# tsai0507/PolishPathPlanning

Measured on AMD Instinct MI355X. Metric: polishing waypoints/sec for 1M-pt cloud, 256 slices; path L2 err vs ref, higher is better.
Workload: dtype f32; 1 GPU; cfg2_1m_s256; points_per_workpiece=999912, slices=256, waypoints_per_workpiece=25908, workpieces=1, batch_per_gpu=1, parallelism=single GPU, pairing=kd, walk=center_int (connect), dynamic_adjustment=False, handles_taking_turns=3

## Files before the change

### polishpathplanning_amd/csrc/ppp_engine.hip

```cpp
#include "ppp_kernels.h"
#ifdef PPP_SINGLE_TU
#include "ppp_window.h"
#endif
#include "ppp_handle.h"
#include "ppp_gather.h"
#include <atomic>
#include <cerrno>
#include <fcntl.h>
#include <thread>
#include <unistd.h>
#ifndef PPP_NN_HINT_SPACINGS
#define PPP_NN_HINT_SPACINGS 3.0
#endif
#ifndef PPP_SLAB_PTS
#define PPP_SLAB_PTS 832
#endif
#ifndef PPP_PPT8_FROM
#define PPP_PPT8_FROM 500000
#endif
#ifndef WIN_SLICE_WAVES_PER_CU
#define WIN_SLICE_WAVES_PER_CU 16
#endif
#ifndef PPP_WIN_PPT8_FROM
#define PPP_WIN_PPT8_FROM 1200000
// ... 324 lines not shown
    if (!capw) return PPP_OK;
    h->win_NBc_thr = std::max(16, NBc / 2);
    while (h->win_NBc_thr * 2 <= NBc && h->win_NBc_thr < expect / 10.0) h->win_NBc_thr <<= 1;
    if (const char *ev = tuning_env("PPP_WIN_NBC_THR")) { const int v = atoi(ev); if (v >= 16 && v <= NBc && (v & (v - 1)) == 0) h->win_NBc_thr = v; }
    const int NB = WIN_CLASSES * NBc;
    h->win_el_expect = max_el;
    h->win_capw = capw; h->win_cap_el = cap_el; h->win_NB = NB; h->win_NBc = NBc;
    int T = win_pick_threads(h, std::max(1, h->se - h->sb));
    if (!T) return PPP_OK;
    h->win_ppt_alone = n_src > PPP_WIN_PPT8_FROM ? 8 : 4;
    {
        int from = PPP_PPT16_FROM;
        if (const char *ev = tuning_env("PPP_WIN_STAGE_FROM")) from = atoi(ev);
        h->win_staged = n_src > from && !tuning_env("PPP_WIN_NO_STAGE");
    }
    if (h->win_staged) {
        h->win_ppt_alone = 8;
        if (win_scatter_lds_bytes(S, 8, WSC_T, true) + 2048 > (size_t)h->max_lds) h->win_ppt_alone = 4;
        if (win_scatter_lds_bytes(S, h->win_ppt_alone, WSC_T, true) + 2048 > (size_t)h->max_lds) { h->win_staged = false; h->win_ppt_alone = 8; }
    }
    win_pick_scatter(h, std::max(1, h->se - h->sb), n_src);
    h->win_gs = std::max(1, (n_src + h->win_ppt * h->win_scat_threads - 1) / (h->win_ppt * h->win_scat_threads));
    if (h->win_staged) h->win_gs = std::min(h->win_gs, std::max(1, h->num_cus));
    h->win_pad = pad; h->win_capw = capw; h->win_cap_el = cap_el; h->win_NB = NB; h->win_NBc = NBc; h->win_threads = T;
    h->win_stride = std::max(1, (int)per);
    h->win_rec_lds = (h->win_stride <= cap_el / 7) ? cap_el / 7 : 0;
#ifdef WIN_REC_GLOBAL
    h->win_rec_lds = 0;
#endif
    h->win_first_kept = h->P.drop_ends ? 1 : 0;
    h->win_nkept = std::max(0, h->P.drop_ends ? S - 2 : S);
    h->win_px0 = px[0];
    HIPCHK(h, h->win_part.ensure((size_t)std::max(h->win_gs, (n_src + 2 * 256 - 1) / (2 * 256))));
    HIPCHK(h, h->win_pts.ensure((size_t)S * (size_t)capw));
    {
        const double need = (double)S * (double)cap_el;
        if (need > 1.0e9) return PPP_OK;
        h->node_cap = std::max(h->node_cap, (int)need);
        HIPCHK(h, h->node_x.ensure(h->node_cap)); HIPCHK(h, h->node_y.ensure(h->node_cap)); HIPCHK(h, h->node_z.ensure(h->node_cap));
    }
    const size_t slots = (size_t)std::max(1, h->win_nkept) * (size_t)h->win_stride;
    HIPCHK(h, h->wps_xyz.ensure(slots)); HIPCHK(h, h->wps_normal.ensure(slots)); HIPCHK(h, h->wps_nn.ensure(slots)); HIPCHK(h, h->wps_pre.ensure(6 * slots)); HIPCHK(h, h->wps_rec.ensure(4 * slots));
    if (!from_auto && !inherit)
        HIPCHK(h, hipMemsetAsync(h->win_cnt.p, 0, sizeof(int) * (size_t)S * std::max<size_t>(3, WIN_CNT_STRIDE), h->stream));
    h->win_path = true;
    if (!inherit && h->sb == 0 && h->se == S && !h->use_part) {
        h->inh_valid = true; h->inh_S = S; h->inh_n = n_src; h->inh_max_w = max_w; h->inh_max_el = max_el; h->inh_pad = pad; h->inh_P = h->P;
    }
    if (getenv("PPP_WIN_DEBUG"))
        fprintf(stderr, "[ppp] window plan: S %d [%d,%d) pad %.2f capw %d cap_el %d NBc %d (throughput %d) threads %d ppt %d x %d threads lds %zu B max window %d max left side %d census %s\n",
                S, h->sb, h->se, pad, capw, cap_el, NBc, h->win_NBc_thr, T, h->win_ppt, h->win_scat_threads, win_slice_lds_for(h, NBc), max_w, max_el,
                from_auto ? "came with the cloud" : (inherit ? "inherited from an earlier cloud of this size" : "at plan time"));
    return PPP_OK;
}

static WinArgs win_args(const ppp_handle h)
{
    WinArgs A;
    memset(&A, 0, sizeof(A));
    A.m = h->meta.p; A.P = dev_params(h);
    A.X = h->use_part ? h->Xp.p : h->X.p; A.Y = h->use_part ? h->Yp.p : h->Y.p; A.Z = h->use_part ? h->Zp.p : h->Z.p;
    A.idmap = h->use_part ? h->part_idx.p : ((h->part_given && h->part_has_idx) ? h->part_idx.p : nullptr);
    A.n = h->use_part ? h->n_part : (int)h->n;
    A.plan_px = h->win_px.p;
    A.S = h->S_cap; A.sb = h->sb; A.se = h->se; A.first_kept = h->win_first_kept; A.nkept = h->win_nkept;
    A.pad = h->win_pad; A.px0 = h->win_px0; A.inv_step = 1.0f / (float)std::max(1, (int)(h->P.tool_radius * 2));
    A.y0 = h->h_mn[1];
    { const float yr = h->h_mx[1] - h->h_mn[1]; A.yscale = yr > 0.f ? (float)h->win_NBc / yr : 0.f; }
    for (int d = 0; d < 3; ++d) { A.plan_mn[d] = h->h_mn[d]; A.plan_mx[d] = h->h_mx[d]; }
    A.plan_nvalid = h->h_nvalid;
    A.capw = h->win_capw; A.cap_el = h->win_cap_el; A.NB = h->win_NB; A.NBc = h->win_NBc; A.stride = h->win_stride; A.rec_lds = h->win_rec_lds;
    A.W_cap = h->W_cap; A.node_cap = h->node_cap;
    A.g_scatter = h->win_gs; A.g_slice = std::max(0, h->se - h->sb); A.g_finish = h->sm_tiles;
    A.finish = h->ranged ? 0 : 1;
    A.win_cnt = h->win_cnt.p; A.win_pts = h->win_pts.p; A.win_part = h->win_part.p;
    A.px = h->px.p; A.lo = h->lo.p; A.hi = h->hi.p;
    A.node_x = h->node_x.p; A.node_y = h->node_y.p; A.node_z = h->node_z.p;
    A.node_start = h->node_start.p; A.node_cnt = h->node_cnt.p; A.band_cnt = h->band_cnt.p;
    A.wp_cnt = h->wp_cnt.p; A.wp_off = h->wp_off.p; A.tail = h->tail.p;
    A.wps_xyz = h->wps_xyz.p; A.wps_normal = h->wps_normal.p; A.wps_nn = h->wps_nn.p; A.wps_pre = h->wps_pre.p; A.wps_rec = h->wps_rec.p;
    A.wp_pre = h->wp_pre.p; A.wp_smooth = h->wp_smooth.p; A.wp_out = h->wp_out.p; A.out2 = h->out2; A.out2_cap = h->out2_cap;
    A.plan_rec = (h->rec_current && h->plan_walk_ok) ? h->plan_auto.p : nullptr;
    A.meta_host = h->hmeta_pinned.p; A.fin_ticket = h->fin_ticket.p;
    return A;
}
static size_t win_slice_lds(const ppp_handle h) { return win_slice_lds_for(h, h->win_NBc); }
static void win_args_throughput(const ppp_handle h, WinArgs &A)
{
    A.NBc = h->win_NBc_thr; A.NB = WIN_CLASSES * A.NBc;
    const float yr = h->h_mx[1] - h->h_mn[1];
    A.yscale = yr > 0.f ? (float)A.NBc / yr : 0.f;
}

static int enqueue_window_gen(ppp_handle h)
{
    WinArgs A = win_args(h);
    const bool thr = win_throughput_launch(h, A.g_slice);
    if (thr) win_args_throughput(h, A);
    const size_t scat_lds = win_scatter_lds_bytes(A.S, h->win_ppt, h->win_scat_threads, h->win_staged);
    if (h->win_scat_threads != WSC_T) {
        const int rcn = with_narrow_scatter(h->win_scat_threads, h->win_ppt, [&](auto ppt, auto st) -> int {
            LAUNCH(h, "k_win_scatter", (k_win_scatter<decltype(ppt)::value, false, decltype(st)::value>), A.g_scatter, decltype(st)::value, scat_lds, A);
            return PPP_OK;
        });
        if (rcn) return rcn;
    }
    else if (h->win_staged && h->win_ppt == 8) LAUNCH(h, "k_win_scatter", (k_win_scatter<8, true>), A.g_scatter, WSC_T, scat_lds, A);
    else if (h->win_staged) LAUNCH(h, "k_win_scatter", (k_win_scatter<4, true>), A.g_scatter, WSC_T, scat_lds, A);
    else if (h->win_ppt == 8) LAUNCH(h, "k_win_scatter", (k_win_scatter<8, false>), A.g_scatter, WSC_T, scat_lds, A);
    else if (h->win_ppt == 2) LAUNCH(h, "k_win_scatter", (k_win_scatter<2, false>), A.g_scatter, WSC_T, scat_lds, A);
    else LAUNCH(h, "k_win_scatter", (k_win_scatter<4, false>), A.g_scatter, WSC_T, scat_lds, A);
    const int T = h->win_threads;
    const size_t lds = win_slice_lds_for(h, A.NBc);
    const int extra = tuning_env("PPP_WIN_NO_VERIFY") ? 0 : 1;
    return with_block_size(T, [&](auto bs) -> int {
        LAUNCH(h, "k_win_slice", k_win_slice<decltype(bs)::value>, A.g_slice + extra, T, lds, A);
        return PPP_OK;
    });
}
static int enqueue_window_finish(ppp_handle h)
{
    const WinArgs A = win_args(h);
    LAUNCH(h, "k_win_finish", k_win_finish, A.g_finish, SMF_T, sizeof(int) * ((size_t)A.nkept + 2), A);
    return PPP_OK;
}

static int make_plan(ppp_handle h)
{
    if (!h->have_cloud) return fail(h, PPP_ERR_ARG, "no cloud set");
    h->pass.withdraw_plan();
    h->drop_graph();
    const int n = (int)h->n;
    int S = h->h_nvalid ? ppp_slice_walk(h->P.walk, h->h_mn[0], h->h_mx[0], h->P.tool_radius, nullptr, 0) : 0;
    if (S >= PPP_WALK_HARD_MAX) return fail(h, PPP_ERR_CAPACITY, "slice walk does not terminate");
    h->sb = std::min(std::max(0, h->P.slice_begin), S);
    h->se = (h->P.slice_end <= 0 || h->P.slice_end > S) ? S : h->P.slice_end;
    h->ranged = S > 0 && (h->sb > 0 || h->se < S);
    h->incl_lo = -INFINITY; h->incl_hi = INFINITY;
    h->n_range = h->h_nvalid;
    if (h->ranged) {
        if (h->sb >= h->se) { h->incl_lo = INFINITY; h->incl_hi = -INFINITY; h->n_range = 0; }
        else {
            std::vector<float> px((size_t)S);
            ppp_slice_walk(h->P.walk, h->h_mn[0], h->h_mx[0], h->P.tool_radius, px.data(), S);
            h->incl_lo = (float)((int)px[h->sb] - 2) - h->P.range_margin;
            h->incl_hi = (float)((int)px[h->se - 1] + 2) + h->P.range_margin;
            const double range = (double)h->h_mx[0] - (double)h->h_mn[0];
            const double part = std::min((double)h->incl_hi, (double)h->h_mx[0]) - std::max((double)h->incl_lo, (double)h->h_mn[0]);
            h->n_range = range > 0 ? (int)std::min((double)h->h_nvalid, std::max(0.0, part / range) * h->h_nvalid * 1.05 + 64) : h->h_nvalid;
        }
    }
    h->use_part = false; h->n_part = 0;
    if (h->part_given) {
        if (!h->ranged && !(h->part_lo == -INFINITY && h->part_hi == INFINITY))
            return fail(h, PPP_ERR_ARG, "a part-only cloud (ppp_set_cloud_part) needs a slice range: set slice_begin / slice_end");
        if (h->sb < h->se && !(h->incl_lo >= h->part_lo && h->incl_hi <= h->part_hi))
            return fail(h, PPP_ERR_ARG, "the slice range with its margin reaches beyond the part this handle was given (ppp_range_interval tells what it needs)");
        h->n_range = n;
    } else if (h->ranged && h->sb < h->se && n > 0) {
        const int nblocks = (n + COMPACT_CHUNK - 1) / COMPACT_CHUNK;
        DevBuf<int> bcnt;
        hipError_t e = bcnt.ensure((size_t)nblocks + 1);
        if (e != hipSuccess) return fail(h, PPP_ERR_HIP, std::string("range part: ") + hipGetErrorString(e));
        PartSel sel{h->X.p, h->Y.p, h->Z.p, h->incl_lo, h->incl_hi};
        int n_part = 0;
        int rc = compact(h, sel, n, bcnt.p, bcnt.p + nblocks, [&](int kept) -> int {
            const size_t np = (size_t)std::max(kept, 1);
// ... 1 lines not shown
            sel.X2 = h->Xp.p; sel.Y2 = h->Yp.p; sel.Z2 = h->Zp.p; sel.idx2 = h->part_idx.p;
            n_part = kept;
            return PPP_OK;
        });
        if (rc) return rc;
        HIPCHK(h, hipStreamSynchronize(h->stream));
        h->n_part = n_part;
        h->n_range = n_part;
        h->use_part = true;
    }
    const int SLAB_PTS = PPP_SLAB_PTS;
    int B = (h->h_nvalid + SLAB_PTS - 1) / SLAB_PTS;
    B = std::max(1, std::min(B, 8192));
    h->B = B;
    {
        double mean = (double)h->h_nvalid / B;
        h->slab_cap = (int)std::min(4096.0, std::max(1024.0, 128.0 * std::ceil(PPP_SLAB_CAP_FACTOR * mean / 128.0)));
    }
    HIPCHK(h, h->big_slabs.ensure(B));
    h->mm_grid = std::max(1, std::min(((h->use_part ? h->n_part : n) / 4 + 255) / 256, 2048));
    HIPCHK(h, h->mm_part.ensure(h->mm_grid));
    h->S_cap = std::max(1, S);
    HIPCHK(h, h->big_slices.ensure(h->S_cap));
    double range = (double)h->h_mx[0] - (double)h->h_mn[0];
    double expect = range > 0 ? (double)h->h_nvalid * 4.0 / range : (double)h->h_nvalid;
    int capb = (int)std::min(4096.0, std::max(1024.0, 128.0 * std::ceil(2.0 * expect / 128.0)));
    h->capb = capb;
    if (1.2 * expect > 4096 || 1.2 * (double)h->h_nvalid / B > 4096) h->big_path = true;
    if (h->big_path) HIPCHK(h, h->arena.ensure((size_t)64 * (size_t)std::max(n, 1) + (1u << 20)));
    double yr = (double)h->h_mx[1] - (double)h->h_mn[1];
    double per = std::max(0.0, (yr - 2 * h->P.trim)) / h->P.path_resolution + 2.0;
    {
        {
            int kc = 256;
            while (kc < capb && kc < 0.75 * expect) kc <<= 1;
            h->knot_cap = kc;
        }
        h->pose_pad = h->P.dynamic_adjustment ? 8.f : std::max(5.f, 2.f * h->P.normal_radius);
        const double slab_w = range > 0 ? range / B : 0.0;
        const double slabs = slab_w > 0 ? std::floor(2.0 * h->pose_pad / slab_w) + 2.0 : 1.0;
        const double want = 1.05 * slabs * ((double)h->h_nvalid / B) + 64;
        h->stage_cap = (int)std::min<double>(POSE_STAGE_CAP, std::max(512.0, 128.0 * std::ceil(want / 128.0)));
        h->tab_slabs = (int)std::min(16.0, slabs);
        while (pose_lds_bytes(h->knot_cap, h->stage_cap, h->tab_slabs) > (size_t)h->max_lds - 8192 && h->knot_cap > 256) h->knot_cap >>= 1;
        while (pose_lds_bytes(h->knot_cap, h->stage_cap, h->tab_slabs) > (size_t)h->max_lds - 8192 && h->stage_cap > 512) h->stage_cap -= 128;
        h->cnt_est = (int)std::min(1.0e6, per);
        h->pose_threads = std::min(POSE_T, std::max(256, 64 * ((h->cnt_est * pose_lanes(h->cnt_est) + 63) / 64)));
    }
    double wc = per * (double)h->S_cap;
    if (wc > 2.0e8) return fail(h, PPP_ERR_CAPACITY, "waypoint bound too large");
    h->W_cap = std::max(1, (int)wc);
    int step = (int)(h->P.tool_radius * 2);
    double overlap = step >= 5 ? 1.0 : 5.0 / std::max(1, step) + 1.0;
    h->node_cap = std::max(16, (int)std::min(2.0e9, overlap * (double)n + 16));

    HIPCHK(h, h->unsorted4.ensure(n)); HIPCHK(h, h->sorted4.ensure(n));
    const int *slab_cnt_before = h->slab_cnt.p;
    HIPCHK(h, h->slab_cnt.ensure(B)); HIPCHK(h, h->slab_start.ensure(B + 1)); HIPCHK(h, h->slab_cursor.ensure(B));
    HIPCHK(h, h->coarse_cursor.ensure((B >> SCAT_COARSE_SHIFT) + 2));
    HIPCHK(h, h->slab_ytab.ensure((size_t)B * (YTB + 1)));
    if (h->ranged || h->part_given) HIPCHK(h, hipMemsetAsync(h->slab_ytab.p, 0, (size_t)B * (YTB + 1) * sizeof(int), h->stream));
    h->two_pass_scatter = B >= 4096 && h->n_range >= 3000000;
    if (h->slab_cnt_used || h->slab_cnt.p != slab_cnt_before) {
        HIPCHK(h, hipMemsetAsync(h->slab_cnt.p, 0, sizeof(int) * (size_t)B, h->stream));
        h->slab_cnt_used = false;
    }
    HIPCHK(h, h->slab_xmin.ensure(B)); HIPCHK(h, h->slab_xmax.ensure(B));
    HIPCHK(h, h->px.ensure(h->S_cap)); HIPCHK(h, h->lo.ensure(h->S_cap)); HIPCHK(h, h->hi.ensure(h->S_cap));
    if (h->P.dynamic_adjustment) {
        h->dyn_maxNB = (int)std::min(4.0e6, std::max(0.0, yr - 4) / (h->P.tool_radius / 4) + 4);
        h->dyn_maxNA = (int)std::min(4.0e6, yr / 5 + 4);
        h->node_cap = (int)std::min(2.0e9, (double)h->node_cap + (double)h->S_cap * h->dyn_maxNA);
        int rc = ensure_dynamic_buffers(h);
        if (rc) return rc;
    }
    HIPCHK(h, h->node_x.ensure(h->node_cap)); HIPCHK(h, h->node_y.ensure(h->node_cap)); HIPCHK(h, h->node_z.ensure(h->node_cap));
    HIPCHK(h, h->node_start.ensure(h->S_cap)); HIPCHK(h, h->node_cnt.ensure(h->S_cap)); HIPCHK(h, h->band_cnt.ensure(h->S_cap));
    HIPCHK(h, h->wp_cnt.ensure(h->S_cap)); HIPCHK(h, h->wp_off.ensure(h->S_cap + 1)); HIPCHK(h, h->tail.ensure(h->S_cap));
    HIPCHK(h, h->slice_wpcnt.ensure(h->S_cap));
    HIPCHK(h, h->wp_xyz.ensure(h->W_cap)); HIPCHK(h, h->wp_normal.ensure(h->W_cap)); HIPCHK(h, h->wp_nn.ensure(h->W_cap));
    HIPCHK(h, h->wp_pre.ensure(6 * (size_t)h->W_cap)); HIPCHK(h, h->wp_smooth.ensure(6 * (size_t)h->W_cap));
    HIPCHK(h, h->wp_out.ensure(6 * (size_t)h->W_cap));
    h->sm_tiles = smooth_tiles(h->W_cap);
    { int rcw = plan_window(h, S, per); if (rcw) return rcw; }
    h->pass.plan_made();
    h->drop_graph();
    return PPP_OK;
}

static int scatter_grid(int n, int ppt) { return std::max(1, (n + ppt * SCAT_T - 1) / (ppt * SCAT_T)); }

SlabGeom slab_geom(const ppp_handle h)
{
    SlabGeom G;
    const int n = h->use_part ? h->n_part : (int)h->n;
    const float xr = h->h_mx[0] - h->h_mn[0];
    G.slab_x0 = h->h_mn[0];
    G.slab_invw = (h->h_nvalid && xr > 0.f) ? (float)h->B / xr : 0.f;
    G.g_minmax = std::max(1, std::min(h->mm_grid, PPP_MM_GRID_MAX));
    G.ppt = (n > PPP_PPT16_FROM && !h->two_pass_scatter) ? 16 : (n > PPP_PPT8_FROM ? 8 : 4);
    G.g_scatter = scatter_grid(n, G.ppt); G.g_scatter2 = scatter_grid(n, 4);
    G.B = h->B; G.slab_cap = h->slab_cap;
    G.full_slabs = h->B > 0 && h->h_nvalid / h->B > 1000;
    G.first_slab = 0; G.g_sort = h->B;
    if (h->use_part && G.slab_invw > 0.f) {
        auto slab_of_host = [&](float x) { int b = (int)((x - G.slab_x0) * G.slab_invw); b = b < 0 ? 0 : b; return b >= h->B ? h->B - 1 : b; };
        G.first_slab = slab_of_host(h->incl_lo);
        G.g_sort = slab_of_host(h->incl_hi) - G.first_slab + 1;
    }
    G.capb = h->capb;
    G.two_fit = 2 * (slice_kd_bytes(h->capb) + 1024) <= (size_t)h->max_lds;
    G.slices = h->S_cap; G.g_slice = h->S_cap; G.g_pose = std::max(1, h->S_cap); G.g_smooth = h->sm_tiles;
    G.pose_threads = h->pose_threads; G.pose_lds = pose_lds_bytes(h->knot_cap, h->stage_cap, h->tab_slabs);
    return G;
}

static SlabArgs slab_args(const ppp_handle h, const SlabGeom &G)
{
    SlabArgs A;
    memset(&A, 0, sizeof(A));
    A.m = h->meta.p; A.P = dev_params(h);
    A.X = h->use_part ? h->Xp.p : h->X.p; A.Y = h->use_part ? h->Yp.p : h->Y.p; A.Z = h->use_part ? h->Zp.p : h->Z.p;
    A.idmap = h->use_part ? h->part_idx.p : ((h->part_given && h->part_has_idx) ? h->part_idx.p : nullptr);
    A.n = h->use_part ? h->n_part : (int)h->n; A.ncloud = (int)h->n;
    A.mm_part = h->mm_part.p;
    A.slab_x0 = G.slab_x0; A.slab_invw = G.slab_invw;
    A.B = h->B; A.S_cap = h->S_cap; A.slab_cap = h->slab_cap; A.capb = h->capb; A.node_cap = h->node_cap; A.W_cap = h->W_cap;
    A.knot_cap = h->knot_cap; A.stage_cap = h->stage_cap; A.tab_slabs = h->tab_slabs; A.pose_pad = h->pose_pad;
    A.first_slab = G.first_slab; A.arena_ran = h->big_path ? 1 : 0;
    A.g_minmax = G.g_minmax; A.g_scatter = G.g_scatter; A.g_sort = G.g_sort; A.g_slice = G.g_slice; A.g_pose = G.g_pose; A.g_smooth = G.g_smooth;
    A.slab_cnt = h->slab_cnt.p; A.slab_start = h->slab_start.p; A.slab_cursor = h->slab_cursor.p; A.coarse_cursor = h->coarse_cursor.p;
    A.px = h->px.p; A.lo = h->lo.p; A.hi = h->hi.p;
    A.unsorted4 = h->unsorted4.p; A.sorted4 = h->sorted4.p; A.slab_xmin = h->slab_xmin.p; A.slab_xmax = h->slab_xmax.p;
    A.big_slabs = h->big_slabs.p; A.big_slices = h->big_slices.p; A.arena = h->arena.p; A.arena_cap = (unsigned long long)h->arena.cap;
    A.node_x = h->node_x.p; A.node_y = h->node_y.p; A.node_z = h->node_z.p;
    A.node_start = h->node_start.p; A.node_cnt = h->node_cnt.p; A.band_cnt = h->band_cnt.p;
    A.wp_cnt = h->wp_cnt.p; A.wp_off = h->wp_off.p; A.tail = h->tail.p;
    A.wp_xyz = h->wp_xyz.p; A.wp_normal = h->wp_normal.p; A.wp_nn = h->wp_nn.p;
    A.wp_pre = h->wp_pre.p; A.wp_smooth = h->wp_smooth.p; A.wp_out = h->wp_out.p; A.out2 = h->out2; A.out2_cap = h->out2_cap;
    A.ytab = h->slab_ytab.p;
    A.slice_wpcnt = (h->P.pairing == PPP_PAIR_KD && !h->P.dynamic_adjustment) ? h->slice_wpcnt.p : nullptr;
    return A;
}

static int enqueue_index(ppp_handle h, const SlabGeom &G, SlabArgs A)
{
    h->slab_cnt_used = true;
    A.P.keep_run_state = (h->win_path && h->pass.gen_done()) ? 1 : 0;
    LAUNCH(h, "k_minmax", k_minmax<true>, A.g_minmax, MM_T, G.hist_lds(), A);
    if (!h->two_pass_scatter) {
        const int rcs = with_ppt(G.ppt, [&](auto ppt) -> int {
            LAUNCH(h, "k_scatter_setup", k_scatter_setup<decltype(ppt)::value>, A.g_scatter + 1, SCAT_T, 2 * G.hist_lds(), A);
            return PPP_OK;
        });
        if (rcs) return rcs;
    } else {
        LAUNCH(h, "k_setup", k_setup, 1, SETUP_T, 0, A);
        LAUNCH(h, "k_slab_scatter", (k_slab_scatter<1, 8>), A.g_scatter, SCAT_T, G.hist_lds(), A);
        LAUNCH(h, "k_slab_scatter2", (k_slab_scatter<2, 4>), G.g_scatter2, SCAT_T, G.hist_lds(), A);
    }
    LAUNCH(h, "k_slab_sort", k_slab_sort<false>, A.g_sort, G.sort_threads(), G.sort_lds(), A);
    if (h->big_path) LAUNCH(h, "k_slab_sort_arena", k_slab_sort<true>, h->B, SORT_T, 0, A);
    h->pass.index_enqueued();
    return PPP_OK;
}

// ... 1886 lines not shown
```

### polishpathplanning_amd/csrc/ppp_handle.h

```cpp
#pragma once
#include "ppp_window_decl.h"
#include "ppp_dynamic.h"
#include "ppp_compact.h"
#include "../../include/ppp_hip.h"
#include <algorithm>
#include <cmath>
#include <cstdlib>
#include <functional>
#include <memory>
#include <string>
#include <vector>

struct RegAcc;
struct FeedRec;

namespace ppp_internal __attribute__((visibility("hidden"))) {

struct KTimer {
    std::string name;
    std::vector<hipEvent_t> e0, e1;
    int used = 0;
};

template <typename T, bool PINNED>
// ... 198 lines not shown
        DevBuf<unsigned char> status;
        DevBuf<unsigned long long> acc;
    } deviation;
    struct Registration {
        DevBuf<double> T;
        DevBuf<unsigned long long> acc;
        DevBuf<ppp_registration_row> rows;
        DevBuf<int> ctl;
    } registration;
    struct ContactField {
        DevBuf<float> curv, hw;
        DevBuf<unsigned long long> acc;
        DevBuf<double> psum;
        bool valid = false;
        unsigned long long built = 0;
        ppp_params P = {};
        float min_width = 0.f;
        ppp_contact_field_stats stats = {};
    } field;
    struct FieldTile {
        DevBuf<float> curv, hw, hw_own;
        DevBuf<unsigned char> owned;
        DevBuf<int> cnt;
        DevBuf<unsigned long long> acc;
        DevBuf<double> psum;
        bool valid = false;
        unsigned long long built = 0;
        ppp_params P = {};
        float halo = 0.f, min_width = 0.f;
        ppp_contact_field_tile_stats stats = {};
    } ftile;
    struct RegionTile {
        bool valid = false;
        int source = -1;
        float threshold = 0.f, link = 0.f;
        unsigned long long serial = 0;
        std::vector<int> labels;
        std::vector<ppp_region_part> parts;
        std::vector<ppp_region_halo> halos;
        ppp_region_tile_stats stats = {};
        DevBuf<unsigned char> owned;
        DevBuf<int> cnt;
    } rtile;
    struct Regions {
        DevBuf<unsigned char> sel, mask;
        DevBuf<int> list, ord, parent, labels, head_root, cnt;
        DevBuf<RegAcc> acc, rows;
        DevBuf<unsigned> tot;
        bool valid = false, nan_centroid = false;
        int source = -1;
        float threshold = 0.f, link = 0.f;
        unsigned long long serial = 0;
        ppp_region_stats stats = {};
    } regions;
    DevBuf<int> node_start, node_cnt, band_cnt;
    DevBuf<int> wp_cnt, wp_off, tail, slice_wpcnt;
    DevBuf<float4> wp_xyz, wp_normal;
    DevBuf<int> wp_nn;
    DevBuf<float> wp_pre, wp_smooth, wp_out;
    DevBuf<MinMaxPart> mm_part;
    DevBuf<int> big_slabs, big_slices;
    DevBuf<char> arena;
    bool big_path = false;
    int mm_grid = 1, sm_tiles = 1;
    DevBuf<char> scratch;
    bool win_allowed = true;
    bool win_disabled = false;
    bool win_path = false;
    bool win_staged = false;
    float win_pad = 4.f;
    int win_NBc_thr = 0;
    int win_capw = 0, win_cap_el = 0, win_NB = 0, win_NBc = 0, win_stride = 1, win_threads = 256, win_ppt = 4, win_gs = 1;
    int win_scat_threads = WSC_T;
    int win_ppt_alone = 4;
    int win_rec_lds = 0;
    int win_nkept = 0, win_first_kept = 0, win_el_expect = 0;
    float win_px0 = 0.f;
    DevBuf<float> win_px;
    DevBuf<int> win_cnt;
    DevBuf<float4> win_pts;
    DevBuf<MinMaxPart> win_part;
    DevBuf<float4> wps_xyz, wps_normal, wps_rec;
    DevBuf<int> fin_ticket;
    DevBuf<int> wps_nn;
    DevBuf<float> wps_pre;

    DevMeta hmeta;
    PinBuf<DevMeta> hmeta_pinned;
    DevBuf<int> plan_ticket;
    DevBuf<PlanAuto> plan_auto;
    bool auto_valid = false;
    bool plan_reuse = true;
    bool inh_valid = false;
    int inh_S = 0, inh_n = 0, inh_max_w = 0, inh_max_el = 0;
    float inh_pad = 0.f;
    ppp_params inh_P;
    bool auto_px_only = false;
    bool plan_inherited = false;
    int auto_S = 0;
    float auto_pad = 0.f;
    bool slab_cnt_used = true;
    PinBuf<char> pin;
    PinBuf<char> pcd_stage[2];
    hipEvent_t pcd_ev[2] = {nullptr, nullptr};
    int side_by_side = 1;
    bool plan_deferred = false, deferred_census = false;
    bool rec_current = false;
    bool plan_walk_ok = false;
    bool chain_calls = false;
    float *out2 = nullptr;
    int out2_cap = 0;
    float *last_out2 = nullptr;
    int last_out2_cap = 0;
    int internal = 0;
    hipGraph_t graph = nullptr;
    hipGraphExec_t graph_exec = nullptr;
    unsigned epoch = 0;
    unsigned graph_epoch_seen = ~0u;
    struct BatchGraph *batches[2] = {nullptr, nullptr};
    int batch_next = 0;
    bool timing = false;
    std::vector<KTimer> timers;

    void drop_graph()
    {
        if (graph_exec) (void)hipGraphExecDestroy(graph_exec);
        if (graph) (void)hipGraphDestroy(graph);
        graph_exec = nullptr; graph = nullptr;
        ++epoch;
    }
    void drop_batch();
    void cloud_replaced(bool under_plan = false)
    {
        if (under_plan) pass.cloud_replaced_under_plan(); else pass.withdraw_plan();
        field.valid = false; ftile.valid = false; rtile.valid = false;
    }
    ~ppp_handle_s()
    {
        (void)hipSetDevice(device);
        drop_graph();
        drop_batch();
        for (int b = 0; b < 2; ++b) if (pcd_ev[b]) (void)hipEventDestroy(pcd_ev[b]);
        for (auto &t : timers) { for (auto e : t.e0) (void)hipEventDestroy(e); for (auto e : t.e1) (void)hipEventDestroy(e); }
        if (stream) (void)hipStreamDestroy(stream);
        if (back) { delete back; back = nullptr; }
    }
};

struct SlabGeom {
    float slab_x0 = 0.f, slab_invw = 0.f;
    int g_minmax = 1, g_scatter = 1, g_scatter2 = 1, g_sort = 1, g_slice = 1, g_pose = 1, g_smooth = 1;
    int first_slab = 0;
    int ppt = 4;
    int B = 1, slab_cap = 2048, capb = 1024;
    bool full_slabs = false;
    bool two_fit = true;
    long long slices = 0;
    int pose_threads = 256;
    size_t pose_lds = 0;
    size_t hist_lds() const { return sizeof(int) * (size_t)B; }
    int sort_threads() const { return full_slabs ? SORT_T : 256; }
    size_t sort_lds() const { return (size_t)slab_cap * 12 + 16; }
    int slice_threads(int num_cus) const { return (two_fit && slices >= 2LL * num_cus) ? 512 : SLICE_KD_T; }
    size_t slice_lds() const { return slice_kd_bytes(capb); }
    size_t brute_lds() const { return slice_lds_bytes(capb); }
    void join(const SlabGeom &o)
// ... 110 lines not shown
```

### polishpathplanning_amd/csrc/ppp_window.h

```cpp
#pragma once
#include "ppp_kernels.h"
#include "ppp_window_decl.h"

template <int PPT, bool STAGED, int T = WSC_T>
__device__ __forceinline__ void win_scatter_body(const WinArgs &A, const int bx)
{
    extern __shared__ __attribute__((aligned(16))) int s_dyn[];
    float *s_px = (float *)s_dyn;
    int *s_cnt = s_dyn + A.S;
    __shared__ int s_scr[17];
    __shared__ float s_mn[3][T / 64], s_mx[3][T / 64];
    __shared__ int s_n[T / 64];
    const int S = A.S, n = A.n;
    const int i0 = bx * (PPT * (int)blockDim.x);
    STAMP_BEGIN();
    float4 p[PPT];
#pragma unroll
    for (int k = 0; k < PPT; ++k) {
        const int i = i0 + threadIdx.x + k * (int)blockDim.x;
        if (i < n) p[k] = make_float4(A.X[i], A.Y[i], A.Z[i], __int_as_float(A.idmap ? A.idmap[i] : i));
        else p[k] = make_float4(NAN, 0.f, 0.f, 0.f);
    }
    for (int s = threadIdx.x; s < S; s += blockDim.x) { s_px[s] = A.plan_px[s]; s_cnt[s] = 0; }
    if (bx == 0 && threadIdx.x == 0) {
// ... 572 lines not shown
#pragma unroll
    for (int e = 0; e < CE; ++e) if (kb[e] >= 0) { const int b = kb[e] & 0x1fff; ckeys[hc[b] + (kb[e] >> 13)] = kr[e]; kb[e] = b; }
    __syncthreads();
#pragma unroll
    for (int e = 0; e < CE; ++e) {
        const int b = kb[e];
        kb[e] = -1;
        if (b >= 0) {
            const int s0 = hc[b], s1 = hc[b + 1];
            if (s1 - s0 > 1) {
                int rank = 0;
                for (int q = s0; q < s1; ++q) rank += ckeys[q] < kr[e] ? 1 : 0;
                kb[e] = s0 + rank;
            }
        }
    }
    __syncthreads();
#pragma unroll
    for (int e = 0; e < CE; ++e) if (kb[e] >= 0) ckeys[kb[e]] = kr[e];
    if (tid == 0) s_m = 0;
    __syncthreads();
    STAMP(6, 4);
    WIN_STOP(4, (int)ckeys[tid % 64]);
    for (int base = 0; base < ncand; base += T) {
        const int j = base + tid;
        const int o0 = s_m;
        int keep = 0;
        float ky = 0.f, kz = 0.f;
        if (j < ncand) {
            const u64 kj = ckeys[j];
            keep = (j == ncand - 1) || (YK_Y(ckeys[j + 1]) != YK_Y(kj));
            if (keep) {
                int best_i = YK_POS(kj);
                int best_idx = brute ? best_i : idx_of(pts[el0 + best_i]);
                for (int q = j - 1; q >= o0 && YK_Y(ckeys[q]) == YK_Y(kj); --q) {
                    const int ci = YK_POS(ckeys[q]);
                    const int id = brute ? ci : idx_of(pts[el0 + ci]);
                    if (id > best_idx) { best_idx = id; best_i = ci; }
                }
                ky = ord2f(YK_Y(kj)); kz = cz[best_i];
            }
        }
        int tot;
        const int pre = block_exscan_w(keep, s_scr, &tot);
        const int o = o0;
        __syncthreads();
        if (keep) knot[o + pre] = make_float2(ky, kz);
        if (tid == 0) s_m = o + tot;
        __syncthreads();
    }
    const int mm = s_m;
    if (tid == 0) {
        int tot = mm;
        int base = s * cap_el;
        if ((long long)base + tot > (long long)A.node_cap) { set_err(m, DERR_CAPACITY, s); base = 0; tot = 0; }
        s_base = base; s_nk = tot;
        A.node_start[s] = base; A.node_cnt[s] = tot;
        if (tot < 3) set_err(m, DERR_SLICE, s);
        int cnt = 0;
        if (kept && tot >= 1) cnt = sample_count((double)knot[0].x, (double)knot[tot - 1].x, P.trim, P.path_resolution, A.stride);
        if (cnt > A.stride) { win_flag(m, WIN_FLAG_OVERFLOW); cnt = 0; }
        if (tot < 3) cnt = 0;
        s_cnt = cnt;
        if (kept) A.wp_cnt[k] = cnt;
    }
    __syncthreads();
    const int nknots = s_nk, cnt = s_cnt;
    STAMP(6, 5);
    WIN_STOP(5, nknots ^ cnt ^ __float_as_int(knot[0].y));
    for (int i = tid; i < nknots; i += T) {
        const float2 kn = knot[i];
        A.node_x[s_base + i] = Px;
        A.node_y[s_base + i] = kn.x;
        A.node_z[s_base + i] = kn.y;
    }
    if (cnt == 0) return;
    auto Yf = [&](int i) { return (double)knot[i].x; };
    auto Zf = [&](int i) { return (double)knot[i].y; };
    const double ystart = (double)knot[0].x + P.trim;
    const double yfirst = (double)knot[0].x, ylast = (double)knot[mm - 1].x;
    const double inv_span = ylast > yfirst ? (double)(mm - 1) / (ylast - yfirst) : 0.0;
    const bool dy_closed_form = sums_exact(ystart, P.path_resolution, (double)cnt);
    float HE[3][3];
    handeye_rotation(P.handeye, HE);
    const int G = ((4 * cnt + T - 1) / T > (2 * cnt + T - 1) / T) ? 2 : 4, gshift = G == 4 ? 2 : 1;
    const int g = tid & (G - 1), per = T >> gshift;
    const int plane_round = G == 4 ? 2 : 4;
    const int rounds = (cnt + per - 1) / per;
    const int per_round = (cnt + rounds - 1) / rounds;
    const bool has_plane_class = s_cs[3] > s_cs[2];
    const float r2 = P.normal_radius * P.normal_radius;
    auto pose_and_store = [&](float *acc, const int count, const bool found, const int bidx, const float4 c0, const float4 q, const int t) {
        const bool finite = q.y == q.y && q.z == q.z;
        float n4[4] = {NAN, NAN, NAN, NAN};
        if (found && count >= 3) {
            const float cntf = (float)count;
            for (int i = 0; i < 9; ++i) acc[i] /= cntf;
            float cov[9];
            cov[0] = acc[0] - acc[6] * acc[6];
            cov[1] = acc[1] - acc[6] * acc[7];
            cov[2] = acc[2] - acc[6] * acc[8];
            cov[4] = acc[3] - acc[7] * acc[7];
            cov[5] = acc[4] - acc[7] * acc[8];
            cov[8] = acc[5] - acc[8] * acc[8];
            cov[3] = cov[1]; cov[6] = cov[2]; cov[7] = cov[5];
            float ev, nn[3];
            pcl_eigen33_smallest<false>(cov, &ev, nn);
            const float eig_sum = cov[0] + cov[4] + cov[8];
            const float curv = eig_sum != 0.f ? fabsf(ev / eig_sum) : 0.f;
            const float vx = P.viewpoint[0] - c0.x, vy = P.viewpoint[1] - c0.y, vz = P.viewpoint[2] - c0.z;
            if (vx * nn[0] + vy * nn[1] + vz * nn[2] < 0) { nn[0] *= -1; nn[1] *= -1; nn[2] *= -1; }
            n4[0] = nn[0]; n4[1] = nn[1]; n4[2] = nn[2]; n4[3] = curv;
        }
        if (!finite) set_err(m, DERR_QUERY, -1);
        float wp[6], rpy[3];
        pose_from_normal(n4, rpy);
        if (P.change_range) { wp[0] = q.x / 1000; wp[1] = q.y / 1000; wp[2] = q.z / 1000; }
        else { wp[0] = q.x; wp[1] = q.y; wp[2] = q.z; }
        wp[3] = rpy[0]; wp[4] = rpy[1]; wp[5] = rpy[2];
        handeye_apply(HE, P.handeye, wp);
        const size_t slot = (size_t)k * A.stride + (size_t)((k & 1) ? (cnt - 1 - t) : t);
        A.wps_xyz[slot] = q;
        A.wps_nn[slot] = found ? bidx : -1;
        A.wps_normal[slot] = make_float4(n4[0], n4[1], n4[2], n4[3]);
#pragma unroll
        for (int d = 0; d < 6; ++d) A.wps_pre[6 * slot + d] = wp[d];
    };
    float *rec_a = cz, *rec_b = (float *)hc;
    const int rcap = A.rec_lds;
    float *rec_g = (float *)(A.wps_rec + 4 * (size_t)k * A.stride);
    auto rec_put = [&](int t, int w, float v) {
        if (rcap) { if (w < 7) rec_a[w * rcap + t] = v; else rec_b[(w - 7) * rcap + t] = v; }
        else rec_g[16 * (size_t)t + w] = v;
    };
    auto rec_get = [&](int t, int w) -> float {
        if (rcap) return w < 7 ? rec_a[w * rcap + t] : rec_b[(w - 7) * rcap + t];
        return rec_g[16 * (size_t)t + w];
    };
    for (int rd = 0; rd < rounds; ++rd) {
        const int lt = tid >> gshift;
        const int t = rd * per_round + lt;
        const bool act = lt < per_round && t < cnt;
        double dy = ystart;
        if (dy_closed_form) dy = ystart + (double)(act ? t : 0) * P.path_resolution;
        else for (int r = 0; r < (act ? t : 0); ++r) dy += P.path_resolution;
        int iv;
        {
            int gi = (int)((dy - yfirst) * inv_span);
            gi = gi < 0 ? 0 : (gi > mm - 2 ? mm - 2 : gi);
            int steps = 0;
            while (gi > 0 && Yf(gi) > dy && steps < 12) { --gi; ++steps; }
            while (gi < mm - 2 && Yf(gi + 1) <= dy && steps < 12) { ++gi; ++steps; }
            iv = gi;
            if (steps >= 12) iv = gsl_bsearch(mm, dy, Yf);
        }
        const double zd = steffen_eval_at(iv, mm, dy, Yf, Zf);
        const float4 q = make_float4((float)(double)Px, (float)dy, (float)zd, 1.f);
        const bool finite = q.y == q.y && q.z == q.z;
        const bool on = act && finite;
        STAMP(6, 6);
        WIN_STOP(6, __float_as_int(q.z) ^ iv);
        float best = P.nn_hint2;
        int bidx = 0x7fffffff, bpos = 0;
        for (int pass = 0; pass < 2; ++pass) {
            for (int round = 0; round <= plane_round; ++round) {
                if (round == plane_round && !has_plane_class) break;
                const int c = win_unit_class(G, round, g);
                const bool up = (g & 1) == 0;
                const bool mine = on && !(round == plane_round && g >= 2);
                if (mine) {
                    const float gap = c == 0 ? q.x - blo : (c == 4 ? bhi - q.x : 0.f);
                    if (!(gap > 0.f && gap * gap > best)) {
                        const int p0 = V.lower_bound(c, q.y);
                        win_walk(V, c, p0, up, [&](const float4 &kk, int at) {
                            const float dyy = q.y - kk.y;
                            if (dyy * dyy > best) return false;
                            const float d = dist2_flann(q.x, q.y, q.z, kk.x, kk.y, kk.z);
                            const int id = idx_of(kk);
                            if (d < best || (d == best && id < bidx)) { best = d; bidx = id; bpos = at; }
                            return true;
                        });
                    }
                }
                for (int o = G >> 1; o > 0; o >>= 1) {
                    const float od = __shfl_xor(best, o, 64);
                    const int oi = __shfl_xor(bidx, o, 64), op = __shfl_xor(bpos, o, 64);
                    if (od < best || (od == best && oi < bidx)) { best = od; bidx = oi; bpos = op; }
                }
            }
            if (__all(bidx != 0x7fffffff || !on)) break;
            best = INFINITY;
        }
        const bool found = on && bidx != 0x7fffffff;
        const float4 bp = found ? pts[bpos] : make_float4(NAN, NAN, NAN, 0.f);
        STAMP(6, 7);
        WIN_STOP(7, bidx ^ __float_as_int(bp.z));
        if (on && g == 0) {
            bool ok = found;
            if (found) {
                const float dq = sqrtf(best) * 1.0001f + 1.0e-4f;
                ok = dq <= A.pad && fabsf(bp.x - Px) + P.normal_radius * 1.0001f + 1.0e-4f <= A.pad;
            }
            if (!ok) win_flag(m, WIN_FLAG_REACH);
        }
        float acc[9] = {0, 0, 0, 0, 0, 0, 0, 0, 0}, pairsum[9] = {0, 0, 0, 0, 0, 0, 0, 0, 0};
        int count = 0, paircnt = 0;
        const float4 c0 = bp;
        for (int round = 0; round <= plane_round; ++round) {
            if (round == plane_round && !has_plane_class) break;
            float a[9] = {0, 0, 0, 0, 0, 0, 0, 0, 0};
            int cn = 0;
            const int c = win_unit_class(G, round, g);
            const bool up = (g & 1) == 0;
            if (found && !(round == plane_round && g >= 2)) {
                const float gap = c == 0 ? c0.x - blo : (c == 4 ? bhi - c0.x : 0.f);
                if (!(gap > 0.f && gap * gap > r2)) {
                    const int p0 = V.lower_bound(c, c0.y);
                    win_walk(V, c, p0, up, [&](const float4 &kk, int) {
                        const float dyy = c0.y - kk.y;
                        if (dyy * dyy > r2) return false;
                        if (dist2_flann(c0.x, c0.y, c0.z, kk.x, kk.y, kk.z) <= r2) {
                            const float x = kk.x - c0.x, y = kk.y - c0.y, z = kk.z - c0.z;
                            a[0] += x * x; a[1] += x * y; a[2] += x * z;
                            a[3] += y * y; a[4] += y * z; a[5] += z * z;
                            a[6] += x; a[7] += y; a[8] += z;
                            cn++;
                        }
                        return true;
                    });
                }
            }
            for (int o = 1; o < G; o <<= 1) {
#pragma unroll
                for (int i = 0; i < 9; ++i) a[i] += __shfl_xor(a[i], o, 64);
                cn += __shfl_xor(cn, o, 64);
            }
            if (G == 2 && round < 4) {
                if ((round & 1) == 0) {
#pragma unroll
                    for (int i = 0; i < 9; ++i) pairsum[i] = a[i];
                    paircnt = cn;
                    continue;
                }
#pragma unroll
                for (int i = 0; i < 9; ++i) a[i] = pairsum[i] + a[i];
                cn = paircnt + cn;
            }
#pragma unroll
            for (int i = 0; i < 9; ++i) acc[i] += a[i];
            count += cn;
        }
        STAMP(6, 8);
        WIN_STOP(8, count ^ __float_as_int(acc[0] + acc[4] + acc[8]));
#ifdef WIN_SPARSE_POSE
        if (act && g == 0) pose_and_store(acc, count, found, bidx, c0, q, t);
#else
        if (act && g == 0) {
#pragma unroll
            for (int w = 0; w < 9; ++w) rec_put(t, w, acc[w]);
            rec_put(t, 9, __int_as_float(found ? count : -1));
            rec_put(t, 10, __int_as_float(bpos));
            rec_put(t, 11, q.y);
            rec_put(t, 12, q.z);
        }
#endif
    }
#ifndef WIN_SPARSE_POSE
    __syncthreads();
    STAMP(6, 9);
    for (int t = tid; t < cnt; t += T) {
        float acc[9];
#pragma unroll
        for (int w = 0; w < 9; ++w) acc[w] = rec_get(t, w);
        const int count = __float_as_int(rec_get(t, 9));
        const bool found = count >= 0;
        const float4 c0 = found ? pts[__float_as_int(rec_get(t, 10))] : make_float4(NAN, NAN, NAN, 0.f);
        pose_and_store(acc, count, found, idx_of(c0), c0, make_float4((float)(double)Px, rec_get(t, 11), rec_get(t, 12), 1.f), t);
    }
#endif
    STAMP(6, 10);
}

__device__ __forceinline__ void win_verify_body(const WinArgs &A)
{
    extern __shared__ __attribute__((aligned(16))) char s_raw[];
    float *s_px = (float *)s_raw;
    float *s_front = s_px + A.S;
    __shared__ float s_mn[3][WSL_T / 64], s_mx[3][WSL_T / 64];
    __shared__ int s_cnt[WSL_T / 64];
    __shared__ int s_S, s_bad;
    DevMeta *m = A.m;
    const DevParams &P = A.P;
    const int T = (int)blockDim.x, tid = (int)threadIdx.x;
    float mn[3] = {INFINITY, INFINITY, INFINITY}, mx[3] = {-INFINITY, -INFINITY, -INFINITY};
    int cnt = 0;
    for (int i = tid; i < A.g_scatter; i += T) {
        const MinMaxPart r = A.win_part[i];
        cnt += r.cnt;
        for (int d = 0; d < 3; ++d) { mn[d] = fminf(mn[d], r.mn[d]); mx[d] = fmaxf(mx[d], r.mx[d]); }
    }
    const int lane = tid & 63, wid = tid >> 6;
    for (int d = 0; d < 3; ++d) { mn[d] = wave_min(mn[d]); mx[d] = wave_max(mx[d]); }
    cnt = wave_sum(cnt);
    if (lane == 0) { for (int d = 0; d < 3; ++d) { s_mn[d][wid] = mn[d]; s_mx[d][wid] = mx[d]; } s_cnt[wid] = cnt; }
    if (tid == 0) s_bad = 0;
    __syncthreads();
    if (tid == 0) {
        int c = 0;
        const int nw = T >> 6;
        for (int w = 0; w < nw; ++w) c += s_cnt[w];
        float rmn[3], rmx[3];
        for (int d = 0; d < 3; ++d) {
            float a = INFINITY, b = -INFINITY;
            for (int w = 0; w < nw; ++w) { a = fminf(a, s_mn[d][w]); b = fmaxf(b, s_mx[d][w]); }
            rmn[d] = c ? a : 3.402823466e+38f;
            rmx[d] = c ? b : -3.402823466e+38f;
        }
        int bad = 0;
        if (P.bounds_given) {
            for (int d = 0; d < 3; ++d) { if (c && (rmn[d] < P.g_mn[d] || rmx[d] > P.g_mx[d])) bad = 1; rmn[d] = P.g_mn[d]; rmx[d] = P.g_mx[d]; }
            c = P.g_nvalid;
        }
        if (A.plan_rec) {
            const PlanAuto R = *A.plan_rec;
            for (int d = 0; d < 3; ++d) if (rmn[d] != R.fin.mn[d] || rmx[d] != R.fin.mx[d]) bad = 1;
            if (c != R.fin.cnt || R.S != A.S || __float_as_int(R.pad) != __float_as_int(A.pad)) bad = 1;
        } else {
            for (int d = 0; d < 3; ++d) if (rmn[d] != A.plan_mn[d] || rmx[d] != A.plan_mx[d]) bad = 1;
            if (c != A.plan_nvalid) bad = 1;
        }
        int S = c ? slice_walk_device(P.walk, rmn[0], rmx[0], P.tool_radius, s_px, A.S, s_front, 2048) : 0;
        if (S != A.S) bad = 1;
        for (int d = 0; d < 3; ++d) { m->mn[d] = rmn[d]; m->mx[d] = rmx[d]; m->mn_ord[d] = f2ord(rmn[d]); m->mx_ord[d] = f2ord(rmx[d]); }
        m->n_valid = c;
        m->S = S > A.S ? A.S : S;
        m->first_kept = P.drop_ends ? 1 : 0;
        { const int Sc = S > A.S ? A.S : S, nk = P.drop_ends ? Sc - 2 : Sc; m->nkept = nk < 0 ? 0 : nk; }
        m->sb = A.sb; m->se = A.se;
        m->incl_lo = P.incl_lo; m->incl_hi = P.incl_hi;
        s_S = S > A.S ? A.S : S;
        if (bad) s_bad = 1;
    }
    __syncthreads();
    const int S = s_S;
    int bad = 0;
    for (int s = tid; s < S; s += T) {
        const float v = s_px[s];
        if (v != A.plan_px[s]) bad = 1;
        const int position = (int)v;
        A.px[s] = v; A.lo[s] = (float)(-2 + position); A.hi[s] = (float)(2 + position);
    }
    if (bad) s_bad = 1;
// ... 271 lines not shown
#pragma unroll
            for (int u = 0; u < WIN_CENSUS_UNROLL; ++u) { const int i = i0 + u * step; xv[u] = i < n ? X[i] : __int_as_float(0x7fc00000); }
#pragma unroll
            for (int u = 0; u < WIN_CENSUS_UNROLL; ++u) win_census_point(xv[u], px, S, px0, inv_step, pad, cw, ce, cr);
        }
        __syncthreads();
        for (int i = threadIdx.x; i < 3 * S; i += blockDim.x)
            if (s_c[i]) atomicAdd(&cnt[i], s_c[i]);
    }
    __syncthreads();
    if (threadIdx.x == 0) {
        __threadfence();
        s_last = atomicAdd(ticket, 1) == (int)gridDim.x - 1;
    }
    __syncthreads();
    if (!s_last) return;
    __threadfence();
    if (valid) {
        for (int i = threadIdx.x; i < 3 * S; i += blockDim.x) { census_host[i] = __hip_atomic_load(&cnt[i], __ATOMIC_RELAXED, __HIP_MEMORY_SCOPE_AGENT); cnt[i] = 0; }
        for (int i = threadIdx.x; i < S; i += blockDim.x) px_host[i] = px[i];
    }
    if (threadIdx.x == 0) {
        PlanAuto r = *plan;
        r.census = valid ? 1 : 0;
        *plan_host = r;
        *ticket = 0;
    }
}

template <int PPT, bool STAGED, int T>
__global__ void __launch_bounds__(T) k_win_scatter(WinArgs A)
{
    static_assert(!STAGED || T == WSC_T, "the staged form is one workgroup of WSC_T threads per CU");
    if (STAGED) win_scatter_staged_loop<PPT>(A, blockIdx.x, A.g_scatter);
    else win_scatter_body<PPT, false, T>(A, blockIdx.x);
}
template <int PPT, bool STAGED, int T>
__global__ void __launch_bounds__(T) k_win_scatter_b(const WinArgs *__restrict__ mem)
{
    static_assert(!STAGED || T == WSC_T, "the staged form is one workgroup of WSC_T threads per CU");
    const WinArgs &A = mem[blockIdx.y];
    if ((int)blockIdx.x >= A.g_scatter) return;
    if (STAGED) win_scatter_staged_loop<PPT>(A, blockIdx.x, A.g_scatter);
    else win_scatter_body<PPT, false, T>(A, blockIdx.x);
}
template <int TMAX>
__global__ void __launch_bounds__(TMAX) k_win_slice(WinArgs A)
{
    if ((int)blockIdx.x == A.g_slice) { win_verify_body(A); return; }
    win_slice_body<TMAX>(A, blockIdx.x);
}
template <int TMAX>
__global__ void __launch_bounds__(TMAX) k_win_slice_b(const WinArgs *__restrict__ mem)
{
    const WinArgs &A = mem[blockIdx.y];
    if ((int)blockIdx.x > A.g_slice) return;
    if ((int)blockIdx.x == A.g_slice) { win_verify_body(A); return; }
    win_slice_body<TMAX>(A, blockIdx.x);
}
__device__ __forceinline__ void win_publish_meta(const WinArgs &A)
{
    if (!A.meta_host) return;
    __shared__ int s_lastw;
    __syncthreads();
    if (threadIdx.x == 0) {
        __builtin_amdgcn_s_waitcnt(0);
        const int grp = (int)blockIdx.x % WIN_FIN_GROUPS;
        const int members = (A.g_finish - grp + WIN_FIN_GROUPS - 1) / WIN_FIN_GROUPS;
        int last = 0;
        if (__hip_atomic_fetch_add(A.fin_ticket + 1 + grp, 1, __ATOMIC_RELAXED, __HIP_MEMORY_SCOPE_AGENT) == members - 1) {
            __hip_atomic_store(A.fin_ticket + 1 + grp, 0, __ATOMIC_RELAXED, __HIP_MEMORY_SCOPE_AGENT);
            const int groups = A.g_finish < WIN_FIN_GROUPS ? A.g_finish : WIN_FIN_GROUPS;
            last = __hip_atomic_fetch_add(A.fin_ticket, 1, __ATOMIC_RELAXED, __HIP_MEMORY_SCOPE_AGENT) == groups - 1;
        }
        s_lastw = last;
    }
    __syncthreads();
    if (!s_lastw) return;
    const int *src = (const int *)A.m;
    int *dst = (int *)A.meta_host;
    for (int q = threadIdx.x; q < (int)(sizeof(DevMeta) / sizeof(int)); q += blockDim.x) dst[q] = __hip_atomic_load(src + q, __ATOMIC_RELAXED, __HIP_MEMORY_SCOPE_AGENT);
    if (threadIdx.x == 0) __hip_atomic_store(A.fin_ticket, 0, __ATOMIC_RELAXED, __HIP_MEMORY_SCOPE_AGENT);
}
__global__ void __launch_bounds__(SMF_T) k_win_finish(WinArgs A) { win_finish_body(A, blockIdx.x); win_publish_meta(A); }
__global__ void __launch_bounds__(SMF_T) k_win_finish_b(const WinArgs *__restrict__ mem)
{
    const WinArgs &A = mem[blockIdx.y];
    if ((int)blockIdx.x >= A.g_finish) return;
    win_finish_body(A, blockIdx.x);
    win_publish_meta(A);
}
```

### polishpathplanning_amd/csrc/ppp_window_decl.h

```cpp
#pragma once
#include "ppp_kernels.h"

enum { WIN_FLAG_OVERFLOW = 1,
       WIN_FLAG_REACH = 2,
       WIN_FLAG_STALE = 4 };
__device__ inline void win_flag(DevMeta *m, int why) { atomicOr(&m->win_flag, why); }

#define WIN_CLASSES 5
#ifndef WIN_CNT_STRIDE
#define WIN_CNT_STRIDE 1
#endif
#ifndef WIN_EMAX
#define WIN_EMAX 8
#endif
#ifndef WIN_CE
#define WIN_CE 4
#endif

struct WinArgs {
    DevMeta *m;
    DevParams P;
    const float *X, *Y, *Z;
    const int *idmap;
    int n;
    const float *plan_px;
    int S, sb, se, first_kept, nkept;
    float pad, px0, inv_step, y0, yscale;
    float plan_mn[3], plan_mx[3];
    int plan_nvalid;
    int capw, cap_el, NB, NBc, stride, W_cap, node_cap;
    int rec_lds;
    int g_scatter, g_slice, g_finish;
    int finish;
    int *win_cnt;
    float4 *win_pts;
    MinMaxPart *win_part;
    float *px, *lo, *hi;
    float *node_x, *node_y, *node_z;
    int *node_start, *node_cnt, *band_cnt;
    int *wp_cnt, *wp_off, *tail;
    float4 *wps_xyz, *wps_normal;
    float4 *wps_rec;
    int *wps_nn;
    float *wps_pre;
    float *wp_pre, *wp_smooth, *wp_out, *out2;
    int out2_cap;
    DevMeta *meta_host;
    int *fin_ticket;
    const PlanAuto *plan_rec;
};

__host__ __device__ inline size_t win_slice_lds_bytes(int capw, int cap_el, int NB)
{
    return (size_t)capw * 16 + (((size_t)NB + 1) * 4 + 15) / 16 * 16 + (size_t)cap_el * 16 + 16;
}

#ifndef WSC_T
#define WSC_T 1024
#endif
__host__ __device__ inline size_t win_scatter_lds_bytes(int S, int ppt, int threads, bool staged)
{
    return staged ? (size_t)12 * S + 16 + (size_t)18 * ppt * threads : (size_t)8 * S;
}
#ifndef WSL_T
#define WSL_T 1024
#endif
#define WIN_FIN_GROUPS 32
#define WIN_S_MAX 8192
#define WIN_AUTO_SCAP 4096

template <int PPT, bool STAGED, int T = WSC_T> __global__ void k_win_scatter(WinArgs A);
template <int PPT, bool STAGED, int T = WSC_T> __global__ void k_win_scatter_b(const WinArgs *__restrict__ mem);
template <int TMAX> __global__ void k_win_slice(WinArgs A);
template <int TMAX> __global__ void k_win_slice_b(const WinArgs *__restrict__ mem);
__global__ void k_win_finish(WinArgs A);
__global__ void k_win_finish_b(const WinArgs *__restrict__ mem);
__global__ void k_win_gather_stage(WinArgs A, float4 *wp_xyz, int *wp_nn, float4 *wp_normal);
template <bool IN_LDS>
__global__ void k_win_census(const float *__restrict__ X, int n, const float *__restrict__ px, int S, float px0, float inv_step, float pad,
                             int *cnt_win, int *cnt_el, int *cnt_er);
__global__ void k_win_census_auto(const float *__restrict__ X, int n, const float *px, const PlanAuto *plan, float inv_step, int *cnt, int *ticket,
                                  PlanAuto *plan_host, float *px_host, int *census_host);
```

Measured before the change: 959.8 million waypoints/s.

## Precompute hand-eye rotation table and hoist spline sampling out of group rounds

The hand-eye rotation matrix is now computed once per plan by a tiny kernel into a device table, and slice threads load the nine entries instead of recomputing trig per thread. Spline sampling (y, z per waypoint) is moved into a separate pass where each thread evaluates distinct waypoints once and stores them in the record buffer. This removes the redundant evaluation across the G threads of each group in the main rounds. It adds a __syncthreads, extra record-buffer traffic, and a host sync when the table is rebuilt.

```diff
diff --git a/polishpathplanning_amd/csrc/ppp_engine.hip b/polishpathplanning_amd/csrc/ppp_engine.hip
--- a/polishpathplanning_amd/csrc/ppp_engine.hip
+++ b/polishpathplanning_amd/csrc/ppp_engine.hip
@@ -430,7 +430,22 @@
     A.wp_pre = h->wp_pre.p; A.wp_smooth = h->wp_smooth.p; A.wp_out = h->wp_out.p; A.out2 = h->out2; A.out2_cap = h->out2_cap;
     A.plan_rec = (h->rec_current && h->plan_walk_ok) ? h->plan_auto.p : nullptr;
     A.meta_host = h->hmeta_pinned.p; A.fin_ticket = h->fin_ticket.p;
+    A.he_tab = h->he_tab.p;
     return A;
+}
+static int ensure_handeye_table(ppp_handle h)
+{
+    if (h->he_tab_valid && memcmp(h->he_tab_for, h->P.handeye, sizeof(h->he_tab_for)) == 0) return PPP_OK;
+    h->he_tab_valid = false;
+    HIPCHK(h, h->he_tab.ensure(9));
+    HandEye6 he;
+    memcpy(he.v, h->P.handeye, sizeof(he.v));
+    hipLaunchKernelGGL(k_handeye_table, dim3(1), dim3(64), 0, h->stream, he, h->he_tab.p);
+    HIPCHK(h, hipGetLastError());
+    HIPCHK(h, hipStreamSynchronize(h->stream));
+    memcpy(h->he_tab_for, h->P.handeye, sizeof(h->he_tab_for));
+    h->he_tab_valid = true;
+    return PPP_OK;
 }
 static size_t win_slice_lds(const ppp_handle h) { return win_slice_lds_for(h, h->win_NBc); }
 static void win_args_throughput(const ppp_handle h, WinArgs &A)
@@ -598,6 +613,7 @@
     HIPCHK(h, h->wp_pre.ensure(6 * (size_t)h->W_cap)); HIPCHK(h, h->wp_smooth.ensure(6 * (size_t)h->W_cap));
     HIPCHK(h, h->wp_out.ensure(6 * (size_t)h->W_cap));
     h->sm_tiles = smooth_tiles(h->W_cap);
+    { int rch = ensure_handeye_table(h); if (rch) return rch; }
     { int rcw = plan_window(h, S, per); if (rcw) return rcw; }
     h->pass.plan_made();
     h->drop_graph();
diff --git a/polishpathplanning_amd/csrc/ppp_handle.h b/polishpathplanning_amd/csrc/ppp_handle.h
--- a/polishpathplanning_amd/csrc/ppp_handle.h
+++ b/polishpathplanning_amd/csrc/ppp_handle.h
@@ -304,6 +304,9 @@
     DevBuf<MinMaxPart> win_part;
     DevBuf<float4> wps_xyz, wps_normal, wps_rec;
     DevBuf<int> fin_ticket;
+    DevBuf<float> he_tab;
+    float he_tab_for[6] = {0, 0, 0, 0, 0, 0};
+    bool he_tab_valid = false;
     DevBuf<int> wps_nn;
     DevBuf<float> wps_pre;
 
diff --git a/polishpathplanning_amd/csrc/ppp_window.h b/polishpathplanning_amd/csrc/ppp_window.h
--- a/polishpathplanning_amd/csrc/ppp_window.h
+++ b/polishpathplanning_amd/csrc/ppp_window.h
@@ -678,7 +678,15 @@
     const double inv_span = ylast > yfirst ? (double)(mm - 1) / (ylast - yfirst) : 0.0;
     const bool dy_closed_form = sums_exact(ystart, P.path_resolution, (double)cnt);
     float HE[3][3];
+    auto handeye_from_plan = [&]() {
+#pragma unroll
+        for (int i = 0; i < 9; ++i) HE[i / 3][i % 3] = A.he_tab[i];
+    };
+#ifdef WIN_HE_PER_THREAD
     handeye_rotation(P.handeye, HE);
+#elif defined(WIN_SPARSE_POSE)
+    handeye_from_plan();
+#endif
     const int G = ((4 * cnt + T - 1) / T > (2 * cnt + T - 1) / T) ? 2 : 4, gshift = G == 4 ? 2 : 1;
     const int g = tid & (G - 1), per = T >> gshift;
     const int plane_round = G == 4 ? 2 : 4;
@@ -733,14 +741,10 @@
         if (rcap) return w < 7 ? rec_a[w * rcap + t] : rec_b[(w - 7) * rcap + t];
         return rec_g[16 * (size_t)t + w];
     };
-    for (int rd = 0; rd < rounds; ++rd) {
-        const int lt = tid >> gshift;
-        const int t = rd * per_round + lt;
-        const bool act = lt < per_round && t < cnt;
+    auto sample_at = [&](const int tt, float &qy, float &qz, int &iv) {
         double dy = ystart;
-        if (dy_closed_form) dy = ystart + (double)(act ? t : 0) * P.path_resolution;
-        else for (int r = 0; r < (act ? t : 0); ++r) dy += P.path_resolution;
-        int iv;
+        if (dy_closed_form) dy = ystart + (double)tt * P.path_resolution;
+        else for (int r = 0; r < tt; ++r) dy += P.path_resolution;
         {
             int gi = (int)((dy - yfirst) * inv_span);
             gi = gi < 0 ? 0 : (gi > mm - 2 ? mm - 2 : gi);
@@ -751,7 +755,42 @@
             if (steps >= 12) iv = gsl_bsearch(mm, dy, Yf);
         }
         const double zd = steffen_eval_at(iv, mm, dy, Yf, Zf);
-        const float4 q = make_float4((float)(double)Px, (float)dy, (float)zd, 1.f);
+        qy = (float)dy; qz = (float)zd;
+    };
+#ifndef WIN_SPLINE_FORM
+#define WIN_SPLINE_FORM 0
+#endif
+#if WIN_SPLINE_FORM == 0
+    int iv_probe = 0;
+    for (int t = tid; t < cnt; t += T) {
+        float qy, qz;
+        sample_at(t, qy, qz, iv_probe);
+        rec_put(t, 11, qy);
+        rec_put(t, 12, qz);
+    }
+    __syncthreads();
+#endif
+    for (int rd = 0; rd < rounds; ++rd) {
+        const int lt = tid >> gshift;
+        const int t = rd * per_round + lt;
+        const bool act = lt < per_round && t < cnt;
+        float qy = 0.f, qz = 0.f;
+#if WIN_SPLINE_FORM == 0
+        const int iv = iv_probe;
+        (void)iv;
+        if (act) { qy = rec_get(t, 11); qz = rec_get(t, 12); }
+#elif WIN_SPLINE_FORM == 1
+        int iv = 0;
+        if (act && g == 0) sample_at(t, qy, qz, iv);
+        {
+            const int first = (tid & 63) & ~(G - 1);
+            qy = __shfl(qy, first, 64); qz = __shfl(qz, first, 64);
+        }
+#else
+        int iv = 0;
+        sample_at(act ? t : 0, qy, qz, iv);
+#endif
+        const float4 q = make_float4((float)(double)Px, qy, qz, 1.f);
         const bool finite = q.y == q.y && q.z == q.z;
         const bool on = act && finite;
         STAMP(6, 6);
@@ -856,14 +895,19 @@
             for (int w = 0; w < 9; ++w) rec_put(t, w, acc[w]);
             rec_put(t, 9, __int_as_float(found ? count : -1));
             rec_put(t, 10, __int_as_float(bpos));
+#if WIN_SPLINE_FORM != 0
             rec_put(t, 11, q.y);
             rec_put(t, 12, q.z);
-        }
 #endif
+        }
+#endif
     }
 #ifndef WIN_SPARSE_POSE
     __syncthreads();
     STAMP(6, 9);
+#ifndef WIN_HE_PER_THREAD
+    if (tid < cnt) handeye_from_plan();
+#endif
     for (int t = tid; t < cnt; t += T) {
         float acc[9];
 #pragma unroll
@@ -1301,6 +1345,13 @@
     for (int q = threadIdx.x; q < (int)(sizeof(DevMeta) / sizeof(int)); q += blockDim.x) dst[q] = __hip_atomic_load(src + q, __ATOMIC_RELAXED, __HIP_MEMORY_SCOPE_AGENT);
     if (threadIdx.x == 0) __hip_atomic_store(A.fin_ticket, 0, __ATOMIC_RELAXED, __HIP_MEMORY_SCOPE_AGENT);
 }
+__global__ void __launch_bounds__(64) k_handeye_table(HandEye6 he, float *tab)
+{
+    if (blockIdx.x != 0 || threadIdx.x != 0) return;
+    float HE[3][3];
+    handeye_rotation(he.v, HE);
+    for (int i = 0; i < 3; ++i) for (int j = 0; j < 3; ++j) tab[3 * i + j] = HE[i][j];
+}
 __global__ void __launch_bounds__(SMF_T) k_win_finish(WinArgs A) { win_finish_body(A, blockIdx.x); win_publish_meta(A); }
 __global__ void __launch_bounds__(SMF_T) k_win_finish_b(const WinArgs *__restrict__ mem)
 {
diff --git a/polishpathplanning_amd/csrc/ppp_window_decl.h b/polishpathplanning_amd/csrc/ppp_window_decl.h
--- a/polishpathplanning_amd/csrc/ppp_window_decl.h
+++ b/polishpathplanning_amd/csrc/ppp_window_decl.h
@@ -48,7 +48,10 @@
     DevMeta *meta_host;
     int *fin_ticket;
     const PlanAuto *plan_rec;
+    const float *he_tab;
 };
+
+struct HandEye6 { float v[6]; };
 
 __host__ __device__ inline size_t win_slice_lds_bytes(int capw, int cap_el, int NB)
 {
@@ -75,6 +78,7 @@
 template <int TMAX> __global__ void k_win_slice_b(const WinArgs *__restrict__ mem);
 __global__ void k_win_finish(WinArgs A);
 __global__ void k_win_finish_b(const WinArgs *__restrict__ mem);
+__global__ void k_handeye_table(HandEye6 he, float *tab);
 __global__ void k_win_gather_stage(WinArgs A, float4 *wp_xyz, int *wp_nn, float4 *wp_normal);
 template <bool IN_LDS>
 __global__ void k_win_census(const float *__restrict__ X, int n, const float *__restrict__ px, int S, float px0, float inv_step, float pad,
```

Result: no change. 968.7 million waypoints/s (median of 6 runs) (+0.9%).
